# zixinz990/quadruped_landing

Measured on AMD Instinct MI355X. Metric: knot-point constraint+Jacobian evals/sec, higher is better.
Workload: dtype f64

## Files before the change

### quadruped_landing_amd/csrc/qln_ilqr_kernels.hip

```cpp
#include "qln_row16.h"

#include <cmath>
#include <cstdlib>
#include <utility>

namespace qln {
namespace {

constexpr int kCUs = 256;
constexpr size_t kLdsPerCU = 160 * 1024;
#ifndef QLN_ALPHAS
#define QLN_ALPHAS 16
#define QLN_ALPHA_STEP 1
#endif
constexpr int kAlphas = QLN_ALPHAS;
constexpr int kAlphaStep = QLN_ALPHA_STEP;
constexpr int kPerTraj = kWave / kAlphas;
constexpr int kIneq = 6;
constexpr int kEnt = 88;
constexpr int kKn = 9;
constexpr int kLd = 17;
constexpr int kKg = 80;
constexpr int kAcB = 64;
constexpr int kAZero = 60;
constexpr int kBZero = 5;
__host__ __device__ constexpr int ac_slot(int row, int col) { return 4 * col + a_slot(row, col); }

enum { KN_W = 0, KN_T0 = 1,  KN_CQ = 7 , KN_ELL = 8 };

__device__ __forceinline__ double act(double t) { return t > 0 ? 1.0 : 0.0; }
template <int I, bool FIRST>
__device__ __forceinline__ void fmac5_row_bcast(double (&u)[5], const double (&K)[5], double dx) {
    static_assert(I >= 0 && I < 16, "a lane of the row");
    if constexpr (FIRST) {
        asm("s_nop 4\n\t"
            "v_fmac_f64_dpp %0, %5, %10 row_newbcast:%11 row_mask:0xf bank_mask:0xf\n\t"
            "v_fmac_f64_dpp %1, %6, %10 row_newbcast:%11 row_mask:0xf bank_mask:0xf\n\t"
            "v_fmac_f64_dpp %2, %7, %10 row_newbcast:%11 row_mask:0xf bank_mask:0xf\n\t"
            "v_fmac_f64_dpp %3, %8, %10 row_newbcast:%11 row_mask:0xf bank_mask:0xf\n\t"
            "v_fmac_f64_dpp %4, %9, %10 row_newbcast:%11 row_mask:0xf bank_mask:0xf"
            : "+v"(u[0]), "+v"(u[1]), "+v"(u[2]), "+v"(u[3]), "+v"(u[4])
            : "v"(K[0]), "v"(K[1]), "v"(K[2]), "v"(K[3]), "v"(K[4]), "v"(dx), "n"(I));
    } else {
        asm("s_nop 1\n\t"
            "v_fmac_f64_dpp %0, %5, %10 row_newbcast:%11 row_mask:0xf bank_mask:0xf\n\t"
            "v_fmac_f64_dpp %1, %6, %10 row_newbcast:%11 row_mask:0xf bank_mask:0xf\n\t"
            "v_fmac_f64_dpp %2, %7, %10 row_newbcast:%11 row_mask:0xf bank_mask:0xf\n\t"
            "v_fmac_f64_dpp %3, %8, %10 row_newbcast:%11 row_mask:0xf bank_mask:0xf\n\t"
            "v_fmac_f64_dpp %4, %9, %10 row_newbcast:%11 row_mask:0xf bank_mask:0xf"
            : "+v"(u[0]), "+v"(u[1]), "+v"(u[2]), "+v"(u[3]), "+v"(u[4])
            : "v"(K[0]), "v"(K[1]), "v"(K[2]), "v"(K[3]), "v"(K[4]), "v"(dx), "n"(I));
    }
}
template <int I0, int NOP>
__device__ __forceinline__ void fmac_row_bcast_8(double& acc, double rec, double v0, double v1, double v2, double v3, double v4,
                                                 double v5, double v6, double v7) {
    static_assert(I0 >= 0 && I0 + 7 < 16, "lanes of the row");
    asm("s_nop %10\n\t"
        "v_fmac_f64_dpp %0, %1, %2 row_newbcast:%11 row_mask:0xf bank_mask:0xf\n\t"
        "v_fmac_f64_dpp %0, %1, %3 row_newbcast:%12 row_mask:0xf bank_mask:0xf\n\t"
        "v_fmac_f64_dpp %0, %1, %4 row_newbcast:%13 row_mask:0xf bank_mask:0xf\n\t"
        "v_fmac_f64_dpp %0, %1, %5 row_newbcast:%14 row_mask:0xf bank_mask:0xf\n\t"
        "v_fmac_f64_dpp %0, %1, %6 row_newbcast:%15 row_mask:0xf bank_mask:0xf\n\t"
        "v_fmac_f64_dpp %0, %1, %7 row_newbcast:%16 row_mask:0xf bank_mask:0xf\n\t"
        "v_fmac_f64_dpp %0, %1, %8 row_newbcast:%17 row_mask:0xf bank_mask:0xf\n\t"
        "v_fmac_f64_dpp %0, %1, %9 row_newbcast:%18 row_mask:0xf bank_mask:0xf"
        : "+v"(acc)
        : "v"(rec), "v"(v0), "v"(v1), "v"(v2), "v"(v3), "v"(v4), "v"(v5), "v"(v6), "v"(v7), "n"(NOP), "n"(I0), "n"(I0 + 1),
          "n"(I0 + 2), "n"(I0 + 3), "n"(I0 + 4), "n"(I0 + 5), "n"(I0 + 6), "n"(I0 + 7));
}
template <int I, int NOP>
__device__ __forceinline__ void fmac_row_bcast_1(double& acc, double rec, double v) {
    asm("s_nop %3\n\tv_fmac_f64_dpp %0, %1, %2 row_newbcast:%4 row_mask:0xf bank_mask:0xf" : "+v"(acc) : "v"(rec), "v"(v), "n"(NOP), "n"(I));
}
__device__ __forceinline__ double stage_ell_row(const double (&cr)[3], const double (&x)[15], const double (&u)[5]) {
    auto hsq = [](double z) { return 0.5 * z * z; };
    double a0 = 0.0, a1 = 0.0;
    fmac_row_bcast_8<0, 4>(a0, cr[0], hsq(x[0]), hsq(x[1]), hsq(x[2]), hsq(x[3]), hsq(x[4]), hsq(x[5]), hsq(x[6]), hsq(x[7]));
    fmac_row_bcast_8<8, 1>(a1, cr[1], x[4], x[5], x[6], x[7], x[8], x[9], x[10], x[11]);
    fmac_row_bcast_8<8, 1>(a0, cr[0], hsq(x[8]), hsq(x[9]), hsq(x[10]), hsq(x[11]), hsq(x[12]), hsq(x[13]), hsq(x[14]), hsq(u[0]));
    fmac_row_bcast_8<0, 1>(a1, cr[1], hsq(u[1]), hsq(u[2]), hsq(u[3]), hsq(u[4]), x[0], x[1], x[2], x[3]);
    fmac_row_bcast_8<0, 1>(a0, cr[2], x[12], x[13], x[14], u[0], u[1], u[2], u[3], u[4]);
    fmac_row_bcast_1<8, 1>(a1, cr[2], 1.0);
    return a0 + a1;
}

template <int... I, class F>
__device__ __forceinline__ void static_for(std::integer_sequence<int, I...>, F&& f) {
    (f(std::integral_constant<int, I>{}), ...);
}
__device__ __forceinline__ double read_lane(double v, int src) {
    const int lo = __builtin_amdgcn_readlane(__double2loint(v), src), hi = __builtin_amdgcn_readlane(__double2hiint(v), src);
    return __hiloint2double(hi, lo);
}

struct StageIn {
    const double* rec;
    const double* lam5;
    double rho, w;
    bool has_u;
    bool ineq;
    bool q6;
    bool final_ctrl;
    bool terminal;
    double lam_fc;
    const double* lam_term;
    const double* xf;
    double mbg, lb, th_lo, th_hi;
};
struct StageOut {
    double val;
    double ell;
    double t[kIneq];
    double g[kIneq];
    double cq;
    double e_fc;
    double viol;
};

template <bool ELL_GIVEN = false>
__device__ __forceinline__ void stage_eval(const StageIn& I, const double (&x)[15], const double (&u)[5], StageOut& o, double ell_in = 0.0) {
    double ell = ell_in;
    if constexpr (!ELL_GIVEN) {
        ell = I.rec[40];
#pragma unroll
        for (int i = 0; i < 15; ++i) ell += (0.5 * (I.rec[i] * x[i])) * x[i] + I.rec[20 + i] * x[i];
        if (I.has_u) {
#pragma unroll
            for (int i = 0; i < 5; ++i) ell += (0.5 * (I.rec[15 + i] * u[i])) * u[i] + I.rec[35 + i] * u[i];
        }
    }
    o.ell = ell;
    double val = I.w * ell;
    double viol = 0.0;
    if (I.ineq && (I.lam5[0] > 0 || I.lam5[1] > 0 || !(x[1] > I.lb / 2))) {
        double sth, cth;
        sincos(x[2], &sth, &cth);
        o.g[0] = -(x[1] - I.lb / 2 * sth);
        o.g[1] = -(x[1] + I.lb / 2 * sth);
        o.cq = (I.lb / 2) * cth;
    } else {
        o.g[0] = o.g[1] = I.lb / 2 - x[1];
        o.cq = 0.0;
    }
    o.g[2] = x[2] - I.th_hi;
    o.g[3] = I.th_lo - x[2];
    o.g[4] = -x[1];
    o.g[5] = -x[3];
#pragma unroll
    for (int j = 0; j < kIneq; ++j) {
        const bool on = I.ineq && (j < 4 || I.q6);
        const double l = I.lam5[j];
        const double t = on ? fmax(0.0, l + I.rho * o.g[j]) : 0.0;
        o.t[j] = t;
        if (on) {
            val += (t * t - l * l) / (2 * I.rho);
            viol = fmax(viol, o.g[j]);
        }
    }
    o.e_fc = 0.0;
    if (I.final_ctrl) {
        o.e_fc = u[1] + u[3] + I.mbg;
        val += I.lam_fc * o.e_fc + 0.5 * I.rho * o.e_fc * o.e_fc;
        viol = fmax(viol, fabs(o.e_fc));
    }
    if (I.terminal) {
#pragma unroll
        for (int i = 0; i < 14; ++i) {
            const double e = x[i] - I.xf[i];
            val += I.lam_term[i] * e + 0.5 * I.rho * e * e;
            viol = fmax(viol, fabs(e));
        }
    }
    o.val = val;
    o.viol = viol;
}

struct FastStep {
    double imb, imf, iIb, g;
};
__device__ __forceinline__ void step_fast(const FastStep& C, int k, int kt, int im, const double (&x)[15], const double (&u)[5],
                                          double (&xn)[15]) {
    const KnotMode md = knot_mode(k + 1, kt - 1, im);
    const double m1 = md.f1free ? 1.0 : 0.0, m2 = md.f2free ? 1.0 : 0.0;
    const double h = u[4], h2 = h * h, hh2 = 0.5 * h2, h3_6 = h2 * h * (1.0 / 6.0), h4_24 = h2 * h2 * (1.0 / 24.0);
    const double abx = (u[0] + u[2]) * C.imb, aby = (u[1] + u[3]) * C.imb + C.g;
    const double a1x = m1 * (-u[0] * C.imf), a1y = m1 * (-u[1] * C.imf + C.g);
    const double a2x = m2 * (-u[2] * C.imf), a2y = m2 * (-u[3] * C.imf + C.g);
    const double r1x = x[3] - x[0], r1y = x[4] - x[1], r2x = x[5] - x[0], r2y = x[6] - x[1];
    const double w1x = m1 * x[10] - x[7], w1y = m1 * x[11] - x[8], w2x = m2 * x[12] - x[7], w2y = m2 * x[13] - x[8];
    const double tau0 = r1x * u[1] - r1y * u[0] + r2x * u[3] - r2y * u[2];
    const double tauv = w1x * u[1] - w1y * u[0] + w2x * u[3] - w2y * u[2];
    const double taua = C.g * ((1.0 - m1) * u[0] + (1.0 - m2) * u[2]);
    xn[0] = x[0] + h * x[7] + hh2 * abx;
    xn[1] = x[1] + h * x[8] + hh2 * aby;
    xn[2] = x[2] + h * x[9] + C.iIb * (hh2 * tau0 + h3_6 * tauv + h4_24 * taua);
    xn[3] = x[3] + m1 * (h * x[10]) + hh2 * a1x;
    xn[4] = x[4] + m1 * (h * x[11]) + hh2 * a1y;
    xn[5] = x[5] + m2 * (h * x[12]) + hh2 * a2x;
    xn[6] = x[6] + m2 * (h * x[13]) + hh2 * a2y;
    xn[7] = x[7] + h * abx;
    xn[8] = x[8] + h * aby;
    xn[9] = x[9] + C.iIb * (h * tau0 + hh2 * tauv + h3_6 * taua);
    xn[10] = x[10] + h * a1x;
    xn[11] = x[11] + h * a1y;
    xn[12] = x[12] + h * a2x;
    xn[13] = x[13] + h * a2y;
    xn[14] = x[14] + h;
    if (md.jump) {
        xn[4] = 0.0;
        xn[6] = 0.0;
        xn[10] = xn[11] = xn[12] = xn[13] = 0.0;
    }
}

__host__ __device__ constexpr void b_rows(int j, int (&rows)[6]) {
    rows[0] = j & 1;
    rows[1] = 2;
    rows[2] = 3 + j;
    rows[3] = 7 + (j & 1);
    rows[4] = 9;
    rows[5] = 10 + j;
}
constexpr bool b_structure_ok() {
    for (int r = 0; r < 15; ++r)
        for (int j = 0; j < 4; ++j) {
            int rows[6] = {0, 0, 0, 0, 0, 0};
            b_rows(j, rows);
            bool in = false;
            for (int q = 0; q < 6; ++q) in = in || rows[q] == r;
            if (step_union_present(r, 15 + j) && !in) return false;
        }
    return true;
}
static_assert(b_structure_ok(), "the sparse products of the Riccati sweep cover every possible non-zero of a force column");
static_assert(!step_union_present(1, 15), "the zero slot of the B image is outside the union pattern");

struct Lds {
    double *X, *U, *K, *leq, *kn, *P, *A, *B, *T, *S, *Qxx, *Qux, *Quu, *g, *Hd;
    int* map;
};

struct Carved {
    Lds L;
    size_t doubles;
};
__host__ __device__ __forceinline__ Carved carve(double* base, int N) {
    size_t off = 0;
    Carved cv;
    Lds& t = cv.L;
#define QLN_TAKE(field, n)                 \
    t.field = base ? base + off : nullptr; \
    off += (size_t)(((n) + 1) & ~1);
    QLN_TAKE(P, 15 * kLd)
    QLN_TAKE(A, 300)
    t.B = t.A ? t.A + kAcB : nullptr;
    QLN_TAKE(T, 15 * kLd)
    QLN_TAKE(Qxx, 15 * kLd)
    QLN_TAKE(S, 5 * kLd)
    t.K = t.S;
    QLN_TAKE(Qux, 5 * kLd)
    QLN_TAKE(Quu, 26)
    QLN_TAKE(g, 20)
    QLN_TAKE(Hd, 20)
    QLN_TAKE(X, 15 * N)
    QLN_TAKE(U, 5 * N)
    QLN_TAKE(leq, 16)
    QLN_TAKE(kn, kKn * N)
    double* mp = base ? base + off : nullptr;
    off += (size_t)((kStepUnion / 2 + 2 + 1) & ~1);
    t.map = reinterpret_cast<int*>(mp);
#undef QLN_TAKE
    cv.doubles = off;
    return cv;
}

}

size_t ilqr_lds_bytes(int32_t N) { return carve(nullptr, N).doubles * sizeof(double); }
size_t ilqr_scratch_doubles(int32_t B, int32_t N) { return (size_t)B * ((size_t)N * (kEnt + kKg + kIneq) + (size_t)kAlphas * 20 * (size_t)N); }

namespace {

template <int OCC>
__global__ __launch_bounds__(kWave, OCC) void k_al_ilqr(BatchParams P, SolveParams S, double* __restrict__ Zio,
                                                      double* __restrict__ info, double* __restrict__ scratch) {
    extern __shared__ double lds[];
    const int lane = threadIdx.x;
    const int b = xcd_contiguous_index(blockIdx.x, P.B);
    if (b >= P.B) return;
    const int N = P.N;
    const ProblemDesc pd = P.desc[b];
    const int kt = pd.k_trans, im = pd.init_mode;
    const Model M(P);
    const double mbg = P.mb * P.g;
    const double p_lb = P.lb;
    FastStep FS;
    FS.imb = 1.0 / P.mb, FS.imf = 1.0 / P.mf, FS.iIb = 1.0 / M.Ib, FS.g = P.g;
    const double h_lo = S.h_lo, h_hi = S.h_hi, th_lo = S.th_lo, th_hi = S.th_hi, h_prox = S.h_prox;
    const double mu0 = S.mu0, mu_min = S.mu_min, mu_max = S.mu_max, tol = S.tol, inner_tol = S.inner_tol;
    const double rho_factor = S.rho_factor, rho_max = S.rho_max;
    const int max_outer = S.max_outer, max_inner = S.max_inner;
    const bool q6 = S.q6 != 0, exact_h = S.exact_h != 0;
    const Lds L = carve(lds, N).L;
    double* __restrict__ Zb = Zio + (int64_t)b * P.z_stride;
    double* __restrict__ ent = scratch + (int64_t)b * ((int64_t)N * (kEnt + kKg + kIneq) + (int64_t)kAlphas * 20 * N);
    double* __restrict__ Kg = ent + (int64_t)N * kEnt;
    double* __restrict__ traj = Kg + (int64_t)N * kKg;
    double* __restrict__ lamg = traj + (int64_t)kAlphas * 20 * N;
    const double* __restrict__ costg = P.cost + (P.cost_batch > 1 ? (int64_t)b * N * 41 : 0);
    const double* __restrict__ x0g = P.bnd + (int64_t)b * 30;

    {
        for (int i = lane; i < 5 * (N - 1); i += kWave) {
            const int k = i / 5, j = i - 5 * k;
            double v = Zb[20 * k + 15 + j];
            if (j == 4) v = fmin(fmax(v, h_lo), h_hi);
            L.U[i] = v;
        }
        for (int i = lane; i < kIneq * N; i += kWave) lamg[i] = 0.0;
        if (lane < 16) L.leq[lane] = 0.0;
        if (lane < 15) L.X[lane] = x0g[lane];
        for_each_step_entry([lane, map = L.map](auto row, auto col) {
            constexpr int pos_ = step_union_pos(row, col);
            if (lane == (pos_ & 63)) map[pos_] = (col < 15) ? ac_slot(row, col) : kAcB + 5 * row + (col - 15);
        });
    }
    wave_lds_sync();
    double xf[15];
#pragma unroll
    for (int i = 0; i < 15; ++i) xf[i] = x0g[15 + i];

    auto stage_in = [=](int k, double rho, double w) {
        StageIn I;
        I.rec = costg + 41 * k;
        I.lam5 = lamg + kIneq * k;
        I.rho = rho;
        I.w = w;
        I.has_u = k < N - 1;
        I.ineq = k >= 1;
        I.q6 = q6;
        I.final_ctrl = (k == N - 2);
        I.terminal = (k == N - 1);
        I.lam_fc = L.leq[14];
        I.lam_term = L.leq;
        I.xf = xf;
        I.mbg = mbg;
        I.lb = p_lb;
        I.th_lo = th_lo;
        I.th_hi = th_hi;
        return I;
    };

    {
        double x[15], u[5], xn[15];
#pragma unroll
        for (int i = 0; i < 15; ++i) x[i] = L.X[i];
        for (int k = 0; k < N - 1; ++k) {
#pragma unroll
            for (int j = 0; j < 5; ++j) u[j] = L.U[5 * k + j];
            step_forward(M, k, kt, im, x, u, xn);
#pragma unroll
            for (int i = 0; i < 15; ++i) x[i] = xn[i];
            if (lane == 0) {
#pragma unroll
                for (int i = 0; i < 15; ++i) L.X[15 * (k + 1) + i] = xn[i];
            }
        }
    }
    wave_lds_sync();

    unsigned long long tk_refresh = 0, tk_blocks = 0, tk_sweep = 0, tk_roll = 0, tk_accept = 0, tk0;
#define QLN_TICK(acc) do { const unsigned long long t_ = __builtin_amdgcn_s_memtime(); acc += t_ - tk0; tk0 = t_; } while (0)
#ifdef QLN_ROLL_STAMPS
    unsigned long long rl0 = 0;
#define QLN_ROLL_BEGIN() rl0 = __builtin_amdgcn_s_memtime()
#define QLN_ROLL_TICK(acc) do { const unsigned long long t_ = __builtin_amdgcn_s_memtime(); acc += t_ - rl0; rl0 = t_; } while (0)
#else
#define QLN_ROLL_BEGIN() do {} while (0)
#define QLN_ROLL_TICK(acc) do {} while (0)
#endif
#ifdef QLN_SWEEP_STAMPS
    unsigned long long sw0 = 0;
#define QLN_SWEEP_BEGIN() sw0 = __builtin_amdgcn_s_memtime()
#define QLN_SWEEP_TICK(acc) do { const unsigned long long t_ = __builtin_amdgcn_s_memtime(); acc += t_ - sw0; sw0 = t_; } while (0)
#define QLN_ITER_TICK(acc) do { tk0 = __builtin_amdgcn_s_memtime(); } while (0)
#elif defined(QLN_ROLL_STAMPS)
#define QLN_SWEEP_BEGIN() do {} while (0)
#define QLN_SWEEP_TICK(acc) do {} while (0)
#define QLN_ITER_TICK(acc) do { tk0 = __builtin_amdgcn_s_memtime(); } while (0)
#else
#define QLN_SWEEP_BEGIN() do {} while (0)
#define QLN_SWEEP_TICK(acc) do {} while (0)
#define QLN_ITER_TICK(acc) QLN_TICK(acc)
#endif
    double rho = S.rho0, mu = mu0;
    double prev_viol = INFINITY;
    double J_cur = 0.0, viol = INFINITY, last_alpha = 0.0;
    int outer = 0, iters = 0, status = 1;

    auto refresh = [=](double rho, double& J, double& vmax) {
        double Jl = 0.0, vl = 0.0;
        for (int k0 = 0; k0 < N; k0 += kWave) {
            const int k = k0 + lane;
            if (k < N) {
                double x[15], u[5] = {0, 0, 0, 0, 0};
#pragma unroll
                for (int i = 0; i < 15; ++i) x[i] = L.X[15 * k + i];
                if (k < N - 1) {
#pragma unroll
                    for (int j = 0; j < 5; ++j) u[j] = L.U[5 * k + j];
                }
                const double w = (k < N - 1) ? u[4] : 1.0;
                StageIn I = stage_in(k, rho, w);
                StageOut o;
                stage_eval(I, x, u, o);
                double* kn = L.kn + kKn * k;
                kn[KN_W] = w;
#pragma unroll
                for (int j = 0; j < kIneq; ++j) {
                    kn[KN_T0 + j] = o.t[j];
                }
                kn[KN_CQ] = o.cq;
                kn[KN_ELL] = o.ell;
                if (k == N - 2) L.leq[15] = L.leq[14] + rho * o.e_fc;
                Jl += o.val;
                vl = fmax(vl, o.viol);
            }
        }
        J = wave_sum(Jl);
        vmax = wave_max(vl);
        wave_lds_sync();
    };

    refresh(rho, J_cur, viol);
    const int total_outer = max_outer + S.rescue_outer;
    int rescued = 0;
    for (outer = 0; outer < total_outer; ++outer) {
        const bool rescue = outer >= max_outer;
        if (outer == max_outer) {
            rho = fmin(rho, 1e6);
            prev_viol = INFINITY;
            rescued = 1;
        }
        const int inner_cap = rescue ? 60 : max_inner;
        mu = mu0;
        bool stalled = false;
        for (int it = 0; it < inner_cap; ++it) {
            tk0 = __builtin_amdgcn_s_memtime();
            refresh(rho, J_cur, viol);
            ++iters;
            QLN_ITER_TICK(tk_refresh);
            for (int k0 = 0; k0 < N - 1; k0 += kWave) {
                const int k = k0 + lane;
                if (k < N - 1) {
                    const double* zk = L.X + 15 * k;
                    double x[14];
#pragma unroll
                    for (int i = 0; i < 14; ++i) x[i] = zk[i];
                    const double* uk = L.U + 5 * k;
                    const StepBlock blk = step_block(x, uk[0], uk[1], uk[2], uk[3], uk[4], knot_mode(k + 1, kt - 1, im), M);
                    double* e = ent + (int64_t)k * kEnt;
                    for_each_rollout_entry(blk, [&](auto row, auto col, double val) {
                        constexpr int pos_ = step_union_pos(row, col);
                        e[pos_] = val;
                    });
                }
            }
            __threadfence();
            wave_lds_sync();
            QLN_ITER_TICK(tk_blocks);

            bool pd_ok = true;
            {
                const int k = N - 1;
                const double* kn = L.kn + kKn * k;
                const double* rec = costg + 41 * k;
                for (int e = lane; e < 15 * kLd; e += kWave) L.P[e] = 0.0;
                wave_lds_sync();
                if (lane < 15) {
                    const int i = lane;
                    const double xi = L.X[15 * k + i];
                    double gi = rec[i] * xi + rec[20 + i];
                    double hi = rec[i];
                    if (i < 14) {
                        gi += L.leq[i] + rho * (xi - xf[i]);
                        hi += rho;
                    }
                    if (i == 1) {
                        gi += -kn[KN_T0 + 0] - kn[KN_T0 + 1] - kn[KN_T0 + 4];
                        hi += rho * (act(kn[KN_T0 + 0]) + act(kn[KN_T0 + 1]) + act(kn[KN_T0 + 4]));
                    }
                    if (i == 2) {
                        gi += (kn[KN_T0 + 0] - kn[KN_T0 + 1]) * kn[KN_CQ] + kn[KN_T0 + 2] - kn[KN_T0 + 3];
                        hi += rho * ((act(kn[KN_T0 + 0]) + act(kn[KN_T0 + 1])) * kn[KN_CQ] * kn[KN_CQ] + act(kn[KN_T0 + 2]) + act(kn[KN_T0 + 3]));
                    }
                    if (i == 3) {
                        gi += -kn[KN_T0 + 5];
                        hi += rho * act(kn[KN_T0 + 5]);
                    }
                    L.T[kLd * i + 15] = gi;
                    L.P[(kLd + 1) * i] = hi;
                }
                if (lane == 0) {
                    const double off = -rho * (act(kn[KN_T0 + 0]) - act(kn[KN_T0 + 1])) * kn[KN_CQ];
                    L.P[kLd * 1 + 2] = off;
                    L.P[kLd * 2 + 1] = off;
                }
                wave_lds_sync();
            }
            for (int e = lane; e < 300; e += kWave) L.A[e] = 0.0;
            double pf_e0, pf_e1, pf_D, pf_d;
            auto prefetch = [=](int k, double& e0, double& e1, double& cD, double& cd) {
                const double* e = ent + (int64_t)k * kEnt;
                e0 = e[lane];
                e1 = e[min(lane + 64, kStepUnion - 1)];
                const double* rec = costg + 41 * k;
                cD = rec[min(lane, 19)];
                cd = rec[20 + min(lane, 19)];
            };
            prefetch(N - 2, pf_e0, pf_e1, pf_D, pf_d);
            const int m0 = L.map[lane], m1 = L.map[min(lane + 64, kStepUnion - 1)];
            auto stage_knot = [=](int k, int ln, double v0, double v1, double recD, double recd) {
                L.A[m0] = v0;
                L.A[m1] = v1;
                const double* kn = L.kn + kKn * k;
                const double w = kn[KN_W];
                const double t0 = kn[KN_T0 + 0], t1 = kn[KN_T0 + 1], t2 = kn[KN_T0 + 2], t3 = kn[KN_T0 + 3], t4 = kn[KN_T0 + 4],
                             t5 = kn[KN_T0 + 5], cq = kn[KN_CQ], ell = kn[KN_ELL];
                const double lfc = L.leq[15];
                const int i = min(ln, 19);
                const double zi = *((i < 15) ? L.X + 15 * k + i : L.U + 5 * k + (i - 15));
                double gi = w * (recD * zi + recd);
                double hi = w * recD;
                const bool live = k >= 1;
                const double g1 = gi + (-t0 - t1 - t4), h1 = hi + rho * (act(t0) + act(t1) + act(t4));
                const double g2 = gi + ((t0 - t1) * cq + t2 - t3), h2 = hi + rho * ((act(t0) + act(t1)) * cq * cq + act(t2) + act(t3));
                const double g3 = gi + -t5, h3 = hi + rho * act(t5);
                gi = (live && i == 1) ? g1 : (live && i == 2) ? g2 : (live && i == 3) ? g3 : gi;
                hi = (live && i == 1) ? h1 : (live && i == 2) ? h2 : (live && i == 3) ? h3 : hi;
                const bool fc = (k == N - 2) && (i == 16 || i == 18);
                gi = fc ? gi + lfc : gi;
                hi = fc ? hi + rho : hi;
                gi = (exact_h && i == 19) ? gi + ell : gi;
                *((ln < 20) ? L.g + i : L.T + (ln & 7)) = gi;
                *((ln < 20) ? L.Hd + i : L.T + kLd + (ln & 7)) = hi;
            };
            stage_knot(N - 2, lane, pf_e0, pf_e1, pf_D, pf_d);
            if (N >= 3) prefetch(N - 3, pf_e0, pf_e1, pf_D, pf_d);
            wave_lds_sync();
            for (int k = N - 2; k >= 0 && pd_ok; --k) {
                int ln = lane;
#ifndef QLN_HOIST_OCC2
                if constexpr (OCC == 2) asm volatile("" : "+v"(ln));
#endif
                QLN_SWEEP_BEGIN();
                const double* kn = L.kn + kKn * k;
                const double v0 = pf_e0, v1 = pf_e1, recD = pf_D, recd = pf_d;
                if (k > 1) prefetch(k - 2, pf_e0, pf_e1, pf_D, pf_d);
                QLN_SWEEP_TICK(tk_refresh);
                const double h12 = (k >= 1) ? -rho * (act(kn[KN_T0 + 0]) - act(kn[KN_T0 + 1])) * kn[KN_CQ] : 0.0;
                const double hfc = (k == N - 2) ? rho : 0.0;
                constexpr bool kStoresLast = (OCC == 1);
                {
                    const int c = ln & 15, cp = a_coupling(c);
                    const bool cv = c < 15;
                    const int cc = cv ? c : 0;
                    const int cq = max(cp, 0);
                    const double* acp = L.A + 4 * c;
                    const double a0 = acp[0], a2 = acp[1], a9 = acp[2], ac = acp[3];
                    double tv[4];
#pragma unroll
                    for (int it = 0; it < 4; ++it) {
                        const double* pr = L.P + kLd * min((ln >> 4) + 4 * it, 14);
                        tv[it] = fma(pr[cq], ac, fma(pr[9], a9, fma(pr[2], a2, pr[cc] * a0)));
                    }
                    auto store_T = [&]() {
#pragma unroll
                        for (int it = 0; it < 4; ++it) {
                            const int r = (ln >> 4) + 4 * it;
                            if (r < 15 && cv) L.T[kLd * r + c] = tv[it];
                        }
                    };
                    if constexpr (!kStoresLast) store_T();
                    const int rs = min(ln >> 2, 14), js = ln & 3;
                    const double* ps = L.P + kLd * rs;
                    int rows[6];
                    b_rows(js, rows);
                    double accS = 0.0, ahS = 0.0;
#pragma unroll
                    for (int q = 0; q < 6; ++q) accS = fma(ps[rows[q]], L.B[5 * rows[q] + js], accS);
#pragma unroll
                    for (int t = 0; t < 4; ++t) {
                        const int i = js + 4 * t, ic = min(i, 14);
                        const double bv = L.B[(i < 15) ? 5 * i + 4 : kBZero];
                        ahS = fma(ps[ic], bv, ahS);
                    }
                    ahS = quad_sum(ahS);
                    if constexpr (kStoresLast) store_T();
                    if (ln < 60) {
                        L.S[5 * rs + js] = accS;
                        if (js == 0) L.S[5 * rs + 4] = ahS;
                    }
                }
                wave_lds_sync();
                QLN_SWEEP_TICK(tk_blocks);
                {
                    const int c = ln & 15;
                    const double t2 = L.T[2 * kLd + c], t9 = L.T[9 * kLd + c];
                    double qv[4];
#pragma unroll
                    for (int it = 0; it < 4; ++it) {
                        const int r = min((ln >> 4) + 4 * it, 14);
                        const int rp = a_coupling(r), rq = max(rp, 0);
                        const double* arp = L.A + 4 * r;
                        const double a0 = arp[0], a2 = arp[1], a9 = arp[2], ac = arp[3];
                        const double tr = L.T[kLd * r + c], tq = L.T[kLd * rq + c];
                        double acc = *((c == 15) ? L.g + r : (r == c) ? L.Hd + r : L.A + kAZero);
                        if ((r == 1 && c == 2) || (r == 2 && c == 1)) acc += h12;
                        acc = fma(a0, tr, acc);
                        acc = fma(a2, t2, acc);
                        acc = fma(a9, t9, acc);
                        acc = fma(ac, tq, acc);
                        qv[it] = acc;
                    }
                    auto store_Qxx = [&]() {
#pragma unroll
                        for (int it = 0; it < 4; ++it) {
                            const int r = (ln >> 4) + 4 * it;
                            if (r < 15) L.Qxx[kLd * r + c] = qv[it];
                        }
                    };
                    if constexpr (!kStoresLast) store_Qxx();
                    const int jf = (ln >> 4);
                    int rowsf[6];
                    b_rows(jf, rowsf);
                    double quf = *((c == 15) ? L.g + 15 + jf : L.A + kAZero);
#pragma unroll
                    for (int q = 0; q < 6; ++q) quf = fma(L.B[5 * rowsf[q] + jf], L.T[kLd * rowsf[q] + c], quf);
                    if constexpr (!kStoresLast) L.Qux[kLd * jf + c] = quf;
                    const int ch = ln >> 2, p = ln & 3;
                    double quh = 0.0;
#pragma unroll
                    for (int t = 0; t < 4; ++t) {
                        const int i = p + 4 * t, ic = min(i, 14);
                        const double bv = L.B[(i < 15) ? 5 * i + 4 : kBZero];
                        quh = fma(bv, L.T[kLd * ic + ch], quh);
                    }
                    quh = quad_sum(quh) + *((ch == 15) ? L.g + 19 : L.A + kAZero);
                    if constexpr (!kStoresLast) {
                        if (p == 0) L.Qux[4 * kLd + ch] = quh;
                    }
                    const int ju = (ln >> 3) & 3, cu = min(ln & 7, 4);
                    int rowsu[6];
                    b_rows(ju, rowsu);
                    const double hdj = L.Hd[15 + ju], hd19 = L.Hd[19];
                    double quu = (ju == cu) ? hdj + mu : 0.0;
                    if ((ju == 1 && cu == 3) || (ju == 3 && cu == 1)) quu += hfc;
#pragma unroll
                    for (int q = 0; q < 6; ++q) quu = fma(L.B[5 * rowsu[q] + ju], L.S[5 * rowsu[q] + cu], quu);
                    double ahu = 0.0;
#pragma unroll
                    for (int t = 0; t < 4; ++t) {
                        const int i = p + 4 * t, ic = min(i, 14);
                        const double bv = L.B[(i < 15) ? 5 * i + 4 : kBZero];
                        ahu = fma(bv, L.S[5 * ic + 4], ahu);
                    }
                    ahu = quad_sum(ahu);
                    if constexpr (kStoresLast) {
                        store_Qxx();
                        L.Qux[kLd * jf + c] = quf;
                        if (p == 0) L.Qux[4 * kLd + ch] = quh;
                    }
                    if (ln < 32 && (ln & 7) < 5) {
                        L.Quu[5 * ju + cu] = quu;
                        if (cu == 4) L.Quu[20 + ju] = quu;
                    }
                    if (ln == 32) L.Quu[24] = ahu + hd19 + mu + h_prox;
                }
                wave_lds_sync();
                QLN_SWEEP_TICK(tk_sweep);
                stage_knot(max(k - 1, 0), ln, v0, v1, recD, recd);
                double q[5][5], l[5][5], dinv[5];
#pragma unroll
                for (int r = 0; r < 5; ++r)
#pragma unroll
                    for (int c = 0; c < 5; ++c) q[r][c] = L.Quu[5 * r + c];
                double y[5], qu[5];
#pragma unroll
                for (int i = 0; i < 5; ++i) {
                    y[i] = -L.Qux[kLd * i + min(ln, 15)];
                    qu[i] = L.Qux[kLd * i + 15];
                }
                const double hk = L.U[5 * k + 4];
                double vv[5][5];
#pragma unroll
                for (int j = 0; j < 5; ++j) {
                    double dj = q[j][j];
#pragma unroll
                    for (int m = 0; m < j; ++m) dj = fma(-l[j][m], vv[j][m], dj);
                    if (!(dj > 1e-300)) pd_ok = false;
                    double rj = __builtin_amdgcn_rcp(dj);
                    rj = fma(fma(-dj, rj, 1.0), rj, rj);
                    rj = fma(fma(-dj, rj, 1.0), rj, rj);
                    dinv[j] = rj;
#pragma unroll
                    for (int i = j + 1; i < 5; ++i) {
                        double v = q[i][j];
#pragma unroll
                        for (int m = 0; m < j; ++m) v = fma(-l[i][m], vv[j][m], v);
                        vv[i][j] = v;
                        l[i][j] = v * rj;
                    }
                }
                if (!pd_ok) break;
                auto ldl_solve = [&](double (&y)[5], int n) {
#pragma unroll
                    for (int i = 0; i < 5; ++i) {
                        if (i < n) {
#pragma unroll
                            for (int m = 0; m < i; ++m) y[i] = fma(-l[i][m], y[m], y[i]);
                        }
                    }
#pragma unroll
                    for (int i = 0; i < 5; ++i)
                        if (i < n) y[i] *= dinv[i];
#pragma unroll
                    for (int i = 4; i >= 0; --i) {
                        if (i < n) {
#pragma unroll
                            for (int m = i + 1; m < 5; ++m)
                                if (m < n) y[i] = fma(-l[m][i], y[m], y[i]);
                        }
                    }
                };
                ldl_solve(y, 5);
                double dff[5];
#pragma unroll
                for (int i = 0; i < 5; ++i) dff[i] = read_lane(y[i], 15);
                const double lo = h_lo - hk, hi = h_hi - hk;
                const bool clamped = (dff[4] < lo) || (dff[4] > hi);
                if (clamped) {
                    const double hc = fmin(fmax(dff[4], lo), hi);
#pragma unroll
                    for (int i = 0; i < 4; ++i) y[i] = (ln < 15) ? -L.Qux[kLd * i + min(ln, 14)] : -(qu[i] + q[i][4] * hc);
                    y[4] = 0.0;
                    ldl_solve(y, 4);
                    y[4] = 0.0;
#pragma unroll
                    for (int i = 0; i < 4; ++i) dff[i] = read_lane(y[i], 15);
                    dff[4] = hc;
                }
                if (ln < 15) {
#pragma unroll
                    for (int i = 0; i < 5; ++i) L.K[kLd * i + ln] = y[i];
                }
                if (ln < 16) {
#pragma unroll
                    for (int i = 0; i < 5; ++i) Kg[(int64_t)kKg * k + 16 * i + ln] = (ln < 15) ? y[i] : dff[i];
                }
                wave_lds_sync();
                QLN_SWEEP_TICK(tk_roll);
                {
                    const int c = ln & 15;
                    const bool cv = c < 15;
                    const int cc = cv ? c : 0;
                    double qc[5], kcol[5];
#pragma unroll
                    for (int i = 0; i < 5; ++i) {
                        qc[i] = L.Qux[kLd * i + cc];
                        kcol[i] = L.K[kLd * i + cc];
                    }
                    double pv4[4];
#pragma unroll
                    for (int it = 0; it < 4; ++it) {
                        const int r = min((ln >> 4) + 4 * it, 14);
                        double acc = L.Qxx[kLd * r + cc], act_ = L.Qxx[kLd * cc + r];
#pragma unroll
                        for (int i = 0; i < 5; ++i) {
                            acc = fma(L.Qux[kLd * i + r], kcol[i], acc);
                            act_ = fma(qc[i], L.K[kLd * i + r], act_);
                        }
                        pv4[it] = 0.5 * (acc + act_);
                    }
                    auto store_P = [&]() {
#pragma unroll
                        for (int it = 0; it < 4; ++it) {
                            const int r = (ln >> 4) + 4 * it;
                            if (r < 15 && cv) L.P[kLd * r + c] = pv4[it];
                        }
                    };
                    if constexpr (!kStoresLast) store_P();
                    const int lv = min(ln, 14);
                    double pvn = L.Qxx[kLd * lv + 15];
#pragma unroll
                    for (int i = 0; i < 5; ++i) pvn = fma(L.Qux[kLd * i + lv], dff[i], pvn);
                    if constexpr (kStoresLast) store_P();
                    if (ln < 15) L.T[kLd * ln + 15] = pvn;
                }
                wave_lds_sync();
                QLN_SWEEP_TICK(tk_accept);
            }
            if (!pd_ok) {
                mu = fmin(mu * 10.0, mu_max);
                if (mu >= mu_max) {
                    stalled = true;
                    break;
                }
                continue;
            }

            QLN_ITER_TICK(tk_sweep);
            __threadfence();
            double J_try = INFINITY;
            {
                constexpr int kGroups = kPerTraj;
                static_assert(kGroups >= 1 && kGroups * kAlphas * 20 <= 3 * ((15 * kLd + 1) & ~1) + 300 + 2 * ((5 * kLd + 1) & ~1) + 26 + 20 + 20,
                              "the (x, u) slots live in the sweep's matrices, P .. Hd (contiguous in carve())");
                double* const slots = L.P;
                const int a = lane & (kAlphas - 1), grp = lane / kAlphas;
                const double alpha = ldexp(1.0, -a * kAlphaStep);
                double* __restrict__ tz = traj + a;
                double x[15], u[5], xn[15];
                double J = 0.0;
#pragma unroll
                for (int i = 0; i < 15; ++i) x[i] = L.X[i];
                static_assert(kAlphas == 16, "the roll-out lanes are one DPP row");
                double Kr[5], Kn[5];
                auto load_gains = [=](int k, double (&K)[5]) {
                    const double* __restrict__ kp = Kg + (int64_t)kKg * min(k, N - 2) + (lane & 15);
#pragma unroll
                    for (int j = 0; j < 5; ++j) K[j] = kp[16 * j];
                };
                load_gains(0, Kr);
                double lr[kIneq];
                auto fetch_lam = [=](int kk, double (&lo)[kIneq]) {
                    const int kq = min(max(kk, 0), N - 1);
#pragma unroll
                    for (int j = 0; j < kIneq; ++j) lo[j] = lamg[kIneq * kq + j];
                };
                fetch_lam(grp, lr);
                double cr[3];
                auto fetch_rec = [=](int kk, double (&c3)[3]) {
                    const double* __restrict__ r = costg + 41 * min(max(kk, 0), N - 2);
                    c3[0] = r[a];
                    c3[1] = r[16 + a];
                    c3[2] = r[32 + min(a, 8)];
                };
                fetch_rec(grp, cr);
                wave_lds_sync();
                for (int k = 0; k < N - 1; ++k) {
                    QLN_ROLL_BEGIN();
                    load_gains(k + 1, Kn);
                    const int slot = k % kGroups;
                    if (lane < kAlphas) {
#pragma unroll
                        for (int j = 0; j < 5; ++j) u[j] = L.U[5 * k + j] + alpha * row_bcast<15>(Kr[j]);
                        static_for(std::make_integer_sequence<int, 15>{}, [&](auto ic) {
                            constexpr int i = decltype(ic)::value;
                            const double dx = x[i] - L.X[15 * k + i];
                            fmac5_row_bcast<i, i == 0>(u, Kr, dx);
                        });
                        u[4] = fmin(fmax(u[4], h_lo), h_hi);
                        QLN_ROLL_TICK(tk_refresh);
                        double* sl = slots + (slot * kAlphas + a) * 20;
#pragma unroll
                        for (int i = 0; i < 15; ++i) sl[i] = x[i];
#pragma unroll
                        for (int j = 0; j < 5; ++j) {
                            sl[15 + j] = u[j];
                            tz[kAlphas * (20 * k + 15 + j)] = u[j];
                        }
                        step_fast(FS, k, kt, im, x, u, xn);
#pragma unroll
                        for (int i = 0; i < 15; ++i) {
                            x[i] = xn[i];
                            tz[kAlphas * (20 * (k + 1) + i)] = xn[i];
                        }
                    }
                    QLN_ROLL_TICK(tk_blocks);
#pragma unroll
                    for (int j = 0; j < 5; ++j) Kr[j] = Kn[j];
                    wave_lds_sync();
                    QLN_ROLL_TICK(tk_sweep);
                    if (slot == kGroups - 1 || k == N - 2) {
                        const int kb = k - slot, kk = kb + grp;
                        if (kk <= k) {
                            const double* sl = slots + (grp * kAlphas + a) * 20;
                            double xs[15], us[5];
#pragma unroll
                            for (int i = 0; i < 15; ++i) xs[i] = sl[i];
#pragma unroll
                            for (int j = 0; j < 5; ++j) us[j] = sl[15 + j];
                            const double w = exact_h ? us[4] : L.kn[kKn * kk + KN_W];
                            StageIn I = stage_in(kk, rho, w);
                            I.lam5 = lr;
                            StageOut o;
                            stage_eval<true>(I, xs, us, o, stage_ell_row(cr, xs, us));
                            J += o.val;
                        }
                        fetch_lam(kb + kGroups + grp, lr);
                        fetch_rec(kb + kGroups + grp, cr);
                    }
                    QLN_ROLL_TICK(tk_roll);
                }
                if (lane < kAlphas) {
                    double u0[5] = {0, 0, 0, 0, 0};
                    StageIn I = stage_in(N - 1, rho, 1.0);
                    StageOut o;
                    stage_eval(I, x, u0, o);
                    J += o.val;
                }
#pragma unroll
                for (int off = kAlphas; off < kWave; off <<= 1) J += __shfl_xor(J, off, kWave);
                J_try = J;
            }
            QLN_ITER_TICK(tk_roll);
            double J_best = ((lane < kAlphas) && (J_try == J_try) && (J_try < J_cur)) ? J_try : INFINITY;
            int a_star = lane;
#pragma unroll
            for (int off = 32; off > 0; off >>= 1) {
                const double Jo = __shfl_xor(J_best, off, kWave);
                const int ao = __shfl_xor(a_star, off, kWave);
                if (Jo < J_best || (Jo == J_best && ao < a_star)) {
                    J_best = Jo;
                    a_star = ao;
                }
            }
            if (!(J_best < J_cur)) {
                mu = fmin(mu * 10.0, mu_max);
                if (mu >= mu_max) {
                    stalled = true;
                    break;
                }
                continue;
            }
            const double J_new = J_best;
            last_alpha = ldexp(1.0, -a_star * kAlphaStep);
            __threadfence();
            wave_lds_sync();
            {
                const double* __restrict__ tz = traj + a_star;
                for (int i = 15 + lane; i < 20 * (N - 1) + 15; i += kWave) {
                    const int k = i / 20, j = i - 20 * k;
                    const double v = __builtin_nontemporal_load(tz + kAlphas * i);
                    if (j < 15) L.X[15 * k + j] = v;
                    else L.U[5 * k + (j - 15)] = v;
                }
            }
            wave_lds_sync();
            QLN_ITER_TICK(tk_accept);
            mu = fmax(mu / 3.0, mu_min);
            const double dJ = J_cur - J_new;
            if (dJ < inner_tol * (1.0 + fabs(J_new))) break;
        }
        refresh(rho, J_cur, viol);
        if (viol <= tol) {
            status = 0;
            ++outer;
            break;
        }
        for (int k0 = 0; k0 < N; k0 += kWave) {
            const int k = k0 + lane;
            if (k < N && k >= 1) {
#pragma unroll
                for (int j = 0; j < kIneq; ++j) lamg[kIneq * k + j] = L.kn[kKn * k + KN_T0 + j];
            }
        }
        if (lane < 14) L.leq[lane] += rho * (L.X[15 * (N - 1) + lane] - xf[lane]);
        if (lane == 14) L.leq[14] = L.leq[15];
        wave_lds_sync();
        if (viol > 0.25 * prev_viol) rho = fmin(rho * rho_factor, rho_max);
        prev_viol = viol;
        if (stalled && rho >= rho_max) status = 2;
    }

    for (int i = lane; i < 20 * (N - 1); i += kWave) {
        const int k = i / 20, j = i - 20 * k;
        Zb[i] = (j < 15) ? L.X[15 * k + j] : L.U[5 * k + (j - 15)];
    }
    if (lane < 15) Zb[20 * (N - 1) + lane] = L.X[15 * (N - 1) + lane];
    {
        double f = 0.0, hs = 0.0;
        for (int k0 = 0; k0 < N; k0 += kWave) {
            const int k = k0 + lane;
            if (k < N) {
                const double ell = L.kn[kKn * k + KN_ELL];
                const double hk = (k < N - 1) ? L.U[5 * k + 4] : 1.0;
                f += hk * ell;
                if (k < N - 1) hs += hk;
            }
        }
        f = wave_sum(f);
        hs = wave_sum(hs);
        if (info && lane == 0) {
            double* o = info + 16 * (int64_t)b;
            o[0] = (double)outer;
            o[1] = (double)iters;
            o[2] = f;
            o[3] = viol;
            o[4] = rho;
            o[5] = (double)status;
            o[6] = J_cur;
            o[7] = last_alpha;
            o[8] = hs;
            o[9] = mu;
            o[10] = (double)tk_refresh;
            o[11] = (double)tk_blocks;
            o[12] = (double)tk_sweep;
            o[13] = (double)tk_roll;
            o[14] = (double)tk_accept;
            o[15] = (double)rescued;
        }
    }
}

__global__ __launch_bounds__(kWave) void k_exact_rollout(BatchParams P, SolveParams S, double* __restrict__ Zio, double* __restrict__ info) {
    const int b = blockIdx.x * blockDim.x + threadIdx.x;
    if (b >= P.B) return;
    const ProblemDesc pd = P.desc[b];
    const int N = P.N, kt = pd.k_trans, im = pd.init_mode;
    const Model M(P);
    double* __restrict__ Zb = Zio + (int64_t)b * P.z_stride;
    const double* __restrict__ x0g = P.bnd + (int64_t)b * 30;
    const double* __restrict__ costg = P.cost + (P.cost_batch > 1 ? (int64_t)b * N * 41 : 0);
    double x[15], u[5], xn[15];
#pragma unroll
    for (int i = 0; i < 15; ++i) {
        x[i] = x0g[i];
        Zb[i] = x[i];
    }
    double f = 0.0, viol = 0.0, poison = 0.0;
    auto up = [&](double v) {
        viol = fmax(viol, v);
        poison += 0.0 * v;
    };
    auto state_rows = [&](int k, const double (&x)[15]) {
        const double y_init = (im == 1) ? x[4] : x[6], y_other = (im == 1) ? x[6] : x[4];
        up(fabs(y_init));
        if (k + 1 >= kt) up(fabs(y_other));
        up(-(x[1] - (P.lb / 2) * fabs(sin(x[2]))));
        if (k >= 1) {
            up(fmax(x[2] - S.th_hi, S.th_lo - x[2]));
            if (S.q6) up(fmax(-x[1], -x[3]));
        }
    };
    for (int k = 0; k < N - 1; ++k) {
#pragma unroll
        for (int j = 0; j < 5; ++j) u[j] = Zb[20 * k + 15 + j];
        {
            const double* __restrict__ rec = costg + 41 * k;
            double a = (0.5 * (rec[0] * x[0])) * x[0], bb = rec[20] * x[0];
#pragma unroll
            for (int i = 1; i < 15; ++i) {
                a = a + (0.5 * (rec[i] * x[i])) * x[i];
                bb = bb + rec[20 + i] * x[i];
            }
            double cc = (0.5 * (rec[15] * u[0])) * u[0], dd = rec[35] * u[0];
#pragma unroll
            for (int j = 1; j < 5; ++j) {
                cc = cc + (0.5 * (rec[15 + j] * u[j])) * u[j];
                dd = dd + rec[35 + j] * u[j];
            }
            f = f + u[4] * ((((a + bb) + cc) + dd) + rec[40]);
        }
        state_rows(k, x);
        if (k == N - 2) up(fabs(u[1] + u[3] + P.mb * P.g));
        step_forward(M, k, kt, im, x, u, xn);
#pragma unroll
        for (int i = 0; i < 15; ++i) {
            x[i] = xn[i];
            Zb[20 * (k + 1) + i] = xn[i];
        }
    }
    {
        const double* __restrict__ rec = costg + 41 * (N - 1);
        double a = (0.5 * (rec[0] * x[0])) * x[0], bb = rec[20] * x[0];
#pragma unroll
        for (int i = 1; i < 15; ++i) {
            a = a + (0.5 * (rec[i] * x[i])) * x[i];
            bb = bb + rec[20 + i] * x[i];
        }
        f = f + ((a + bb) + rec[40]);
        state_rows(N - 1, x);
#pragma unroll
        for (int i = 0; i < 14; ++i) up(fabs(x[i] - x0g[15 + i]));
    }
    if (poison != poison) viol = poison;
    if (info) {
        info[16 * (int64_t)b + 2] = f;
        info[16 * (int64_t)b + 3] = viol;
    }
}

}

hipError_t launch_al_ilqr(const BatchParams& p, const SolveParams& s, double* Z, double* info, double* scratch, hipStream_t stream) {
    const size_t lds = ilqr_lds_bytes(p.N);
    bool two_per_simd = p.B > 4 * kCUs && 5 * lds <= kLdsPerCU;
#ifdef QLN_TUNING
    if (const char* e = getenv("QLN_ILQR_OCC")) two_per_simd = atoi(e) == 2;
#endif
    auto go = [&](auto kern) {
        hipError_t e = hipFuncSetAttribute(reinterpret_cast<const void*>(kern), hipFuncAttributeMaxDynamicSharedMemorySize, (int)lds);
        if (e != hipSuccess) return e;
        hipLaunchKernelGGL(kern, dim3(xcd_grid(p.B)), dim3(kWave), lds, stream, p, s, Z, info, scratch);
        return hipGetLastError();
    };
    if (hipError_t e2 = two_per_simd ? go(k_al_ilqr<2>) : go(k_al_ilqr<1>); e2 != hipSuccess) return e2;
    hipLaunchKernelGGL(k_exact_rollout, dim3((p.B + kWave - 1) / kWave), dim3(kWave), 0, stream, p, s, Z, info);
    return hipGetLastError();
}

}
```

Measured before the change: 2.524 billion.

## Compute Riccati backward-sweep products with f64 MFMA and register-resident P

Replaces the hand-coded sparse scalar FMA products of the Riccati sweep (T=PA, S=PB, Qxx, Qux, Quu and the P update) with 16x16x4 f64 MFMA instructions. A and B are re-laid out in LDS as MFMA operand images, and P is kept in registers across knots instead of being reread from LDS. This removes the separate K/T/S LDS stages and two wave syncs per knot. The trade-off is that dense MFMAs do work on known-zero entries, and the new operand layout brings correctness risk.

```diff
diff --git a/quadruped_landing_amd/csrc/qln_ilqr_kernels.hip b/quadruped_landing_amd/csrc/qln_ilqr_kernels.hip
--- a/quadruped_landing_amd/csrc/qln_ilqr_kernels.hip
+++ b/quadruped_landing_amd/csrc/qln_ilqr_kernels.hip
@@ -21,10 +21,11 @@
 constexpr int kKn = 9;
 constexpr int kLd = 17;
 constexpr int kKg = 80;
-constexpr int kAcB = 64;
-constexpr int kAZero = 60;
-constexpr int kBZero = 5;
-__host__ __device__ constexpr int ac_slot(int row, int col) { return 4 * col + a_slot(row, col); }
+typedef double d4 __attribute__((ext_vector_type(4)));
+__device__ __forceinline__ d4 mfma_f64(double a, double b, d4 c) { return __builtin_amdgcn_mfma_f64_16x16x4f64(a, b, c, 0, 0, 0); }
+__host__ __device__ constexpr int a_img(int row, int col) { return 4 * (16 * (row & 3) + col) + (row >> 2); }
+__host__ __device__ constexpr int b_img(int row, int j) { return 4 * (5 * (row & 3) + j) + (row >> 2); }
+constexpr int kBZero = 80;
 
 enum { KN_W = 0, KN_T0 = 1,  KN_CQ = 7 , KN_ELL = 8 };
 
@@ -214,30 +215,8 @@
     }
 }
 
-__host__ __device__ constexpr void b_rows(int j, int (&rows)[6]) {
-    rows[0] = j & 1;
-    rows[1] = 2;
-    rows[2] = 3 + j;
-    rows[3] = 7 + (j & 1);
-    rows[4] = 9;
-    rows[5] = 10 + j;
-}
-constexpr bool b_structure_ok() {
-    for (int r = 0; r < 15; ++r)
-        for (int j = 0; j < 4; ++j) {
-            int rows[6] = {0, 0, 0, 0, 0, 0};
-            b_rows(j, rows);
-            bool in = false;
-            for (int q = 0; q < 6; ++q) in = in || rows[q] == r;
-            if (step_union_present(r, 15 + j) && !in) return false;
-        }
-    return true;
-}
-static_assert(b_structure_ok(), "the sparse products of the Riccati sweep cover every possible non-zero of a force column");
-static_assert(!step_union_present(1, 15), "the zero slot of the B image is outside the union pattern");
-
 struct Lds {
-    double *X, *U, *K, *leq, *kn, *P, *A, *B, *T, *S, *Qxx, *Qux, *Quu, *g, *Hd;
+    double *X, *U, *leq, *kn, *P, *A, *B, *T, *S, *Qxx, *Qux, *Quu, *g, *Hd;
     int* map;
 };
 
@@ -254,11 +233,10 @@
     off += (size_t)(((n) + 1) & ~1);
     QLN_TAKE(P, 15 * kLd)
     QLN_TAKE(A, 300)
-    t.B = t.A ? t.A + kAcB : nullptr;
     QLN_TAKE(T, 15 * kLd)
     QLN_TAKE(Qxx, 15 * kLd)
     QLN_TAKE(S, 5 * kLd)
-    t.K = t.S;
+    t.B = t.S;
     QLN_TAKE(Qux, 5 * kLd)
     QLN_TAKE(Quu, 26)
     QLN_TAKE(g, 20)
@@ -321,9 +299,9 @@
         for (int i = lane; i < kIneq * N; i += kWave) lamg[i] = 0.0;
         if (lane < 16) L.leq[lane] = 0.0;
         if (lane < 15) L.X[lane] = x0g[lane];
-        for_each_step_entry([lane, map = L.map](auto row, auto col) {
+        for_each_step_entry([lane, map = L.map, offB = (int)(L.B - L.A)](auto row, auto col) {
             constexpr int pos_ = step_union_pos(row, col);
-            if (lane == (pos_ & 63)) map[pos_] = (col < 15) ? ac_slot(row, col) : kAcB + 5 * row + (col - 15);
+            if (lane == (pos_ & 63)) map[pos_] = (col < 15) ? a_img(row, col) : offB + b_img(row, col - 15);
         });
     }
     wave_lds_sync();
@@ -472,6 +450,7 @@
             QLN_ITER_TICK(tk_blocks);
 
             bool pd_ok = true;
+            d4 Pm;
             {
                 const int k = N - 1;
                 const double* kn = L.kn + kKn * k;
@@ -508,8 +487,15 @@
                     L.P[kLd * 2 + 1] = off;
                 }
                 wave_lds_sync();
-            }
-            for (int e = lane; e < 300; e += kWave) L.A[e] = 0.0;
+#pragma unroll
+                for (int i = 0; i < 4; ++i) {
+                    const int r = (lane >> 4) + 4 * i, rc = min(r, 14), c = lane & 15;
+                    const double v = *((c == 15) ? L.T + kLd * rc + 15 : L.P + kLd * rc + c);
+                    Pm[i] = (r < 15) ? v : 0.0;
+                }
+            }
+            for (int e = lane; e < 256; e += kWave) L.A[e] = 0.0;
+            for (int e = lane; e < kBZero + 4; e += kWave) L.B[e] = 0.0;
             double pf_e0, pf_e1, pf_D, pf_d;
             auto prefetch = [=](int k, double& e0, double& e1, double& cD, double& cd) {
                 const double* e = ent + (int64_t)k * kEnt;
@@ -554,6 +540,8 @@
 #ifndef QLN_HOIST_OCC2
                 if constexpr (OCC == 2) asm volatile("" : "+v"(ln));
 #endif
+                const int r0 = ln >> 4, c = ln & 15;
+                const bool c15 = c == 15;
                 QLN_SWEEP_BEGIN();
                 const double* kn = L.kn + kKn * k;
                 const double v0 = pf_e0, v1 = pf_e1, recD = pf_D, recd = pf_d;
@@ -561,125 +549,44 @@
                 QLN_SWEEP_TICK(tk_refresh);
                 const double h12 = (k >= 1) ? -rho * (act(kn[KN_T0 + 0]) - act(kn[KN_T0 + 1])) * kn[KN_CQ] : 0.0;
                 const double hfc = (k == N - 2) ? rho : 0.0;
-                constexpr bool kStoresLast = (OCC == 1);
-                {
-                    const int c = ln & 15, cp = a_coupling(c);
-                    const bool cv = c < 15;
-                    const int cc = cv ? c : 0;
-                    const int cq = max(cp, 0);
-                    const double* acp = L.A + 4 * c;
-                    const double a0 = acp[0], a2 = acp[1], a9 = acp[2], ac = acp[3];
-                    double tv[4];
-#pragma unroll
-                    for (int it = 0; it < 4; ++it) {
-                        const double* pr = L.P + kLd * min((ln >> 4) + 4 * it, 14);
-                        tv[it] = fma(pr[cq], ac, fma(pr[9], a9, fma(pr[2], a2, pr[cc] * a0)));
-                    }
-                    auto store_T = [&]() {
-#pragma unroll
-                        for (int it = 0; it < 4; ++it) {
-                            const int r = (ln >> 4) + 4 * it;
-                            if (r < 15 && cv) L.T[kLd * r + c] = tv[it];
-                        }
-                    };
-                    if constexpr (!kStoresLast) store_T();
-                    const int rs = min(ln >> 2, 14), js = ln & 3;
-                    const double* ps = L.P + kLd * rs;
-                    int rows[6];
-                    b_rows(js, rows);
-                    double accS = 0.0, ahS = 0.0;
-#pragma unroll
-                    for (int q = 0; q < 6; ++q) accS = fma(ps[rows[q]], L.B[5 * rows[q] + js], accS);
-#pragma unroll
-                    for (int t = 0; t < 4; ++t) {
-                        const int i = js + 4 * t, ic = min(i, 14);
-                        const double bv = L.B[(i < 15) ? 5 * i + 4 : kBZero];
-                        ahS = fma(ps[ic], bv, ahS);
-                    }
-                    ahS = quad_sum(ahS);
-                    if constexpr (kStoresLast) store_T();
-                    if (ln < 60) {
-                        L.S[5 * rs + js] = accS;
-                        if (js == 0) L.S[5 * rs + 4] = ahS;
-                    }
-                }
+                const double* zero = L.B + kBZero;
+                const d4 Am = *reinterpret_cast<const d4*>(L.A + 4 * ln);
+                const d4 Bm = *reinterpret_cast<const d4*>(L.B + 4 * ((c < 5) ? 5 * r0 + c : kBZero / 4));
+                d4 Qxx, Qux = {0.0, 0.0, 0.0, 0.0}, Quu = {0.0, 0.0, 0.0, 0.0};
+#pragma unroll
+                for (int i = 0; i < 4; ++i) {
+                    const int r = r0 + 4 * i;
+                    const double* src = c15 ? ((r < 15) ? L.g + r : zero) : ((r == c) ? L.Hd + r : zero);
+                    Qxx[i] = *src;
+                    if ((r == 1 && c == 2) || (r == 2 && c == 1)) Qxx[i] += h12;
+                }
+                Qux[0] = *(c15 ? L.g + 15 + r0 : zero);
+                Qux[1] = *((c15 && r0 == 0) ? L.g + 19 : zero);
+                Quu[0] = *((r0 == c) ? L.Hd + 15 + r0 : zero) + ((r0 == c) ? mu : 0.0);
+                if ((r0 == 1 && c == 3) || (r0 == 3 && c == 1)) Quu[0] += hfc;
+                Quu[1] = *((ln == 4) ? L.Hd + 19 : zero) + ((ln == 4) ? mu + h_prox : 0.0);
+                d4 Tm = {0.0, 0.0, 0.0, 0.0}, Sm = {0.0, 0.0, 0.0, 0.0};
+#pragma unroll
+                for (int i = 0; i < 4; ++i) Tm = mfma_f64(c15 ? 0.0 : Pm[i], Am[i], Tm);
+#pragma unroll
+                for (int i = 0; i < 4; ++i) Sm = mfma_f64(c15 ? 0.0 : Pm[i], Bm[i], Sm);
+#pragma unroll
+                for (int i = 0; i < 4; ++i) Tm[i] = c15 ? Pm[i] : Tm[i];
+#pragma unroll
+                for (int i = 0; i < 4; ++i) Qxx = mfma_f64(Am[i], Tm[i], Qxx);
+#pragma unroll
+                for (int i = 0; i < 4; ++i) Qux = mfma_f64(Bm[i], Tm[i], Qux);
+#pragma unroll
+                for (int i = 0; i < 4; ++i) Quu = mfma_f64(Bm[i], Sm[i], Quu);
+                if (c < 5 && r0 <= c) {
+                    L.Quu[5 * r0 + c] = Quu[0];
+                    L.Quu[5 * c + r0] = Quu[0];
+                }
+                if (ln == 4) L.Quu[24] = Quu[1];
+                L.Qux[kLd * r0 + c] = Qux[0];
+                if (r0 == 0) L.Qux[kLd * 4 + c] = Qux[1];
                 wave_lds_sync();
                 QLN_SWEEP_TICK(tk_blocks);
-                {
-                    const int c = ln & 15;
-                    const double t2 = L.T[2 * kLd + c], t9 = L.T[9 * kLd + c];
-                    double qv[4];
-#pragma unroll
-                    for (int it = 0; it < 4; ++it) {
-                        const int r = min((ln >> 4) + 4 * it, 14);
-                        const int rp = a_coupling(r), rq = max(rp, 0);
-                        const double* arp = L.A + 4 * r;
-                        const double a0 = arp[0], a2 = arp[1], a9 = arp[2], ac = arp[3];
-                        const double tr = L.T[kLd * r + c], tq = L.T[kLd * rq + c];
-                        double acc = *((c == 15) ? L.g + r : (r == c) ? L.Hd + r : L.A + kAZero);
-                        if ((r == 1 && c == 2) || (r == 2 && c == 1)) acc += h12;
-                        acc = fma(a0, tr, acc);
-                        acc = fma(a2, t2, acc);
-                        acc = fma(a9, t9, acc);
-                        acc = fma(ac, tq, acc);
-                        qv[it] = acc;
-                    }
-                    auto store_Qxx = [&]() {
-#pragma unroll
-                        for (int it = 0; it < 4; ++it) {
-                            const int r = (ln >> 4) + 4 * it;
-                            if (r < 15) L.Qxx[kLd * r + c] = qv[it];
-                        }
-                    };
-                    if constexpr (!kStoresLast) store_Qxx();
-                    const int jf = (ln >> 4);
-                    int rowsf[6];
-                    b_rows(jf, rowsf);
-                    double quf = *((c == 15) ? L.g + 15 + jf : L.A + kAZero);
-#pragma unroll
-                    for (int q = 0; q < 6; ++q) quf = fma(L.B[5 * rowsf[q] + jf], L.T[kLd * rowsf[q] + c], quf);
-                    if constexpr (!kStoresLast) L.Qux[kLd * jf + c] = quf;
-                    const int ch = ln >> 2, p = ln & 3;
-                    double quh = 0.0;
-#pragma unroll
-                    for (int t = 0; t < 4; ++t) {
-                        const int i = p + 4 * t, ic = min(i, 14);
-                        const double bv = L.B[(i < 15) ? 5 * i + 4 : kBZero];
-                        quh = fma(bv, L.T[kLd * ic + ch], quh);
-                    }
-                    quh = quad_sum(quh) + *((ch == 15) ? L.g + 19 : L.A + kAZero);
-                    if constexpr (!kStoresLast) {
-                        if (p == 0) L.Qux[4 * kLd + ch] = quh;
-                    }
-                    const int ju = (ln >> 3) & 3, cu = min(ln & 7, 4);
-                    int rowsu[6];
-                    b_rows(ju, rowsu);
-                    const double hdj = L.Hd[15 + ju], hd19 = L.Hd[19];
-                    double quu = (ju == cu) ? hdj + mu : 0.0;
-                    if ((ju == 1 && cu == 3) || (ju == 3 && cu == 1)) quu += hfc;
-#pragma unroll
-                    for (int q = 0; q < 6; ++q) quu = fma(L.B[5 * rowsu[q] + ju], L.S[5 * rowsu[q] + cu], quu);
-                    double ahu = 0.0;
-#pragma unroll
-                    for (int t = 0; t < 4; ++t) {
-                        const int i = p + 4 * t, ic = min(i, 14);
-                        const double bv = L.B[(i < 15) ? 5 * i + 4 : kBZero];
-                        ahu = fma(bv, L.S[5 * ic + 4], ahu);
-                    }
-                    ahu = quad_sum(ahu);
-                    if constexpr (kStoresLast) {
-                        store_Qxx();
-                        L.Qux[kLd * jf + c] = quf;
-                        if (p == 0) L.Qux[4 * kLd + ch] = quh;
-                    }
-                    if (ln < 32 && (ln & 7) < 5) {
-                        L.Quu[5 * ju + cu] = quu;
-                        if (cu == 4) L.Quu[20 + ju] = quu;
-                    }
-                    if (ln == 32) L.Quu[24] = ahu + hd19 + mu + h_prox;
-                }
-                wave_lds_sync();
-                QLN_SWEEP_TICK(tk_sweep);
                 stage_knot(max(k - 1, 0), ln, v0, v1, recD, recd);
                 double q[5][5], l[5][5], dinv[5];
 #pragma unroll
@@ -689,7 +596,7 @@
                 double y[5], qu[5];
 #pragma unroll
                 for (int i = 0; i < 5; ++i) {
-                    y[i] = -L.Qux[kLd * i + min(ln, 15)];
+                    y[i] = -L.Qux[kLd * i + c];
                     qu[i] = L.Qux[kLd * i + 15];
                 }
                 const double hk = L.U[5 * k + 4];
@@ -743,7 +650,7 @@
                 if (clamped) {
                     const double hc = fmin(fmax(dff[4], lo), hi);
 #pragma unroll
-                    for (int i = 0; i < 4; ++i) y[i] = (ln < 15) ? -L.Qux[kLd * i + min(ln, 14)] : -(qu[i] + q[i][4] * hc);
+                    for (int i = 0; i < 4; ++i) y[i] = !c15 ? -L.Qux[kLd * i + min(c, 14)] : -(qu[i] + q[i][4] * hc);
                     y[4] = 0.0;
                     ldl_solve(y, 4);
                     y[4] = 0.0;
@@ -751,54 +658,29 @@
                     for (int i = 0; i < 4; ++i) dff[i] = read_lane(y[i], 15);
                     dff[4] = hc;
                 }
-                if (ln < 15) {
-#pragma unroll
-                    for (int i = 0; i < 5; ++i) L.K[kLd * i + ln] = y[i];
-                }
+#pragma unroll
+                for (int i = 0; i < 5; ++i) y[i] = c15 ? dff[i] : y[i];
                 if (ln < 16) {
 #pragma unroll
-                    for (int i = 0; i < 5; ++i) Kg[(int64_t)kKg * k + 16 * i + ln] = (ln < 15) ? y[i] : dff[i];
+                    for (int i = 0; i < 5; ++i) Kg[(int64_t)kKg * k + 16 * i + ln] = y[i];
+                }
+                QLN_SWEEP_TICK(tk_roll);
+                const double kd0 = (r0 == 0) ? y[0] : (r0 == 1) ? y[1] : (r0 == 2) ? y[2] : y[3];
+                const double kd1 = (r0 == 0) ? y[4] : 0.0;
+                Qxx = mfma_f64(c15 ? 0.0 : Qux[0], kd0, Qxx);
+                Qxx = mfma_f64(c15 ? 0.0 : Qux[1], kd1, Qxx);
+#pragma unroll
+                for (int i = 0; i < 4; ++i) {
+                    const int r = r0 + 4 * i;
+                    if (r < 15) L.Qxx[kLd * r + c] = Qxx[i];
                 }
                 wave_lds_sync();
-                QLN_SWEEP_TICK(tk_roll);
-                {
-                    const int c = ln & 15;
-                    const bool cv = c < 15;
-                    const int cc = cv ? c : 0;
-                    double qc[5], kcol[5];
-#pragma unroll
-                    for (int i = 0; i < 5; ++i) {
-                        qc[i] = L.Qux[kLd * i + cc];
-                        kcol[i] = L.K[kLd * i + cc];
-                    }
-                    double pv4[4];
-#pragma unroll
-                    for (int it = 0; it < 4; ++it) {
-                        const int r = min((ln >> 4) + 4 * it, 14);
-                        double acc = L.Qxx[kLd * r + cc], act_ = L.Qxx[kLd * cc + r];
-#pragma unroll
-                        for (int i = 0; i < 5; ++i) {
-                            acc = fma(L.Qux[kLd * i + r], kcol[i], acc);
-                            act_ = fma(qc[i], L.K[kLd * i + r], act_);
-                        }
-                        pv4[it] = 0.5 * (acc + act_);
-                    }
-                    auto store_P = [&]() {
-#pragma unroll
-                        for (int it = 0; it < 4; ++it) {
-                            const int r = (ln >> 4) + 4 * it;
-                            if (r < 15 && cv) L.P[kLd * r + c] = pv4[it];
-                        }
-                    };
-                    if constexpr (!kStoresLast) store_P();
-                    const int lv = min(ln, 14);
-                    double pvn = L.Qxx[kLd * lv + 15];
-#pragma unroll
-                    for (int i = 0; i < 5; ++i) pvn = fma(L.Qux[kLd * i + lv], dff[i], pvn);
-                    if constexpr (kStoresLast) store_P();
-                    if (ln < 15) L.T[kLd * ln + 15] = pvn;
-                }
-                wave_lds_sync();
+#pragma unroll
+                for (int i = 0; i < 4; ++i) {
+                    const int r = r0 + 4 * i;
+                    const double mt = L.Qxx[kLd * min(c, 14) + r];
+                    Pm[i] = (r == 15) ? 0.0 : c15 ? Qxx[i] : 0.5 * (Qxx[i] + mt);
+                }
                 QLN_SWEEP_TICK(tk_accept);
             }
             if (!pd_ok) {
```

New measurement: 2.520 billion. Within noise of the previous version (-0.1%).
